# JuliaReinforcementLearning/ReinforcementLearning.jl

Measured on NVIDIA H100. Metric: env-steps/sec at 65536 CartPole envs (full PPO iteration: rollout T=32 + GAE + 4 epochs x 4 minibatches), higher is better.
Workload: dtype f32

## Files before the change

### reinforcementlearning.jl_b200/csrc/nn_tc.cu

```cuda
#include "nn.cuh"
#include "perm.cuh"
#include "policy.cuh"
#include "tc_fwd.cuh"
#include "tc_split.h"
#include "wgmma.cuh"

namespace {

using tcfwd::G_F;
using tcfwd::GW_S;
using tcfwd::WIMG_BYTES;
using tcfwd::split2;
using tcfwd::wimg_off;
constexpr int TM = tcfwd::TM;
constexpr int H = tcfwd::H;
constexpr float kScaleW = tcfwd::kScale;

constexpr int NT7 = 512;
constexpr int kMaxStage = 10;
constexpr int GF_T = 128;
constexpr int GS_T = 16 * GF_T;
constexpr int FIMG = 8 * GS_T;
constexpr float kScaleH = 64.0f, kScaleX = 64.0f;
constexpr int kNo = 2;

struct SmemBwd {
    static_assert(FIMG % 128 == 0 && WIMG_BYTES % 128 == 0 && (2 * GS_T) % 16 == 0, "operand images must stay 128-byte aligned");
    alignas(128) uint8_t FP_full[FIMG];
    alignas(128) uint8_t FP_lo[FIMG];
    alignas(128) uint8_t FH_lo[FIMG];
    alignas(128) uint8_t FH_full[FIMG];
    alignas(128) uint8_t FQ_full[FIMG];
    alignas(128) uint8_t FQ_lo[FIMG];
    alignas(128) uint8_t B1[WIMG_BYTES];
    alignas(128) uint8_t XT[2][2 * GS_T];
    alignas(128) uint8_t AH_full[FIMG];
    alignas(128) uint8_t AH_lo[FIMG];
    alignas(16) float D[TM * H];
    uint64_t H1pos[2][TM];
    float W1[kInMax * H];
    float b1[H], b2[H];
    float W3[H * kNo];
    float b3[kNo];
    float Zp[4 * kNo * TM];
    float Red[32];
    double RedD[16];
    float step_scale;
    alignas(8) uint64_t bar1;
    alignas(8) uint64_t bar3;
    alignas(8) uint64_t bar4;
    float AccW2[64 * 65 + 64];
    float AccD4[64 * 9];
};
__device__ __forceinline__ int d_off(int s, int col) { return s * H + ((((col >> 2) ^ (s & 15))) << 2) + (col & 3); }
__device__ __forceinline__ void d_ld16(const float* D, int s, int f0, float (&v)[16]) {
#pragma unroll
    for (int u = 0; u < 4; ++u) {
        const float4 q4 = *reinterpret_cast<const float4*>(D + d_off(s, f0 + 4 * u));
        v[4 * u] = q4.x; v[4 * u + 1] = q4.y; v[4 * u + 2] = q4.z; v[4 * u + 3] = q4.w;
    }
}
template <int TB>
__device__ __forceinline__ void gemm_ts3(float (&d)[32], const uint8_t* a_hi, const uint8_t* a_lo, int h, uint64_t dB, uint32_t b_step) {
    const uint64_t dA = wg::make_desc(wg::smem_u32(a_hi) + 8 * h * GF_T, GS_T, GF_T), dAl = wg::make_desc(wg::smem_u32(a_lo) + 8 * h * GF_T, GS_T, GF_T);
    wg::fence();
#pragma unroll
    for (int k = 0; k < 4; ++k) {
        const uint32_t aa = k * 2 * GS_T, bb = k * b_step;
        wg::mma_m64n64k16<0, TB>(d, wg::desc_add(dA, aa), wg::desc_add(dB, bb), k ? 1u : 0u);
        wg::mma_m64n64k16<0, TB>(d, wg::desc_add(dA, aa), wg::desc_add(dB, 8 * GW_S + bb), 1u);
        wg::mma_m64n64k16<0, TB>(d, wg::desc_add(dAl, aa), wg::desc_add(dB, bb), 1u);
    }
    wg::commit();
    wg::wait_all();
}
__device__ __forceinline__ uint32_t fimg_off(int f, int s) { return (uint32_t)((f >> 3) * GS_T + (s >> 3) * GF_T + (s & 7) * 16 + (f & 7) * 2); }
__device__ __forceinline__ void store16_feat(uint8_t* img, int f0, int s, const uint32_t (&v)[8]) {
    uint8_t* p = img + fimg_off(f0, s);
    *reinterpret_cast<uint4*>(p) = make_uint4(v[0], v[1], v[2], v[3]);
    *reinterpret_cast<uint4*>(p + GS_T) = make_uint4(v[4], v[5], v[6], v[7]);
}
using b200perm::perm_index;
using b200perm::perm_index_bits;

__device__ __forceinline__ float lane_transpose_reduce32(float (&v)[32], int lane) {
#pragma unroll
    for (int st = 0; st < 5; ++st) {
        const int half = 16 >> st, off = 16 >> st;
        const bool upper = (lane & off) != 0;
#pragma unroll
        for (int n = 0; n < half; ++n) {
            float send = upper ? v[n] : v[n + half];
            float keep = upper ? v[n + half] : v[n];
            v[n] = keep + __shfl_xor_sync(0xffffffffu, send, off);
        }
    }
    return v[0];
}

__device__ __forceinline__ void worker_sync() { asm volatile("bar.sync 1, 512;" ::: "memory"); }
__device__ __forceinline__ void group_sync(int q) { asm volatile("bar.sync %0, 128;" ::"r"(5 + q) : "memory"); }
__device__ __forceinline__ void ready_arrive(int id) { asm volatile("bar.arrive %0, 640;" ::"r"(id) : "memory"); }
__device__ __forceinline__ void ready_wait(int id) { asm volatile("bar.sync %0, 640;" ::"r"(id) : "memory"); }
#ifdef B200RL_K7_TIMING
__device__ unsigned long long g_k7_phase[40];
__device__ int g_k7_watch = 0;
#define K7_T(i) do { if (tid == (g_k7_watch & 0xFFFF) && (int)blockIdx.x == (g_k7_watch >> 16)) { long long now_ = clock64(); g_k7_phase[i] += (unsigned long long)(now_ - tprev_); tprev_ = now_; } } while (0)
#else
#define K7_T(i) do { } while (0)
#endif
constexpr int NT7_ALL = NT7 + 128;
constexpr int kRegsMma = 64, kRegsWorker = 104;
static_assert(128 * kRegsMma + NT7 * kRegsWorker <= NT7_ALL * 96, "setmaxnreg split must fit the CTA's register allocation");
constexpr int kBarRdyA = 2, kBarRdyB = 3;
constexpr int kBarMma = 4;
__device__ __forceinline__ void mma_sync() { asm volatile("bar.sync %0, 128;" ::"n"(kBarMma) : "memory"); }

template <int ACT>
__global__ void __launch_bounds__(NT7_ALL, 1)
ac_loss_grad_tc_kernel(MlpDesc actor, MlpDesc critic, const float* params , AcHyper hp, AcBatch b, float* partial,
                       float* __restrict__ loss_partial, int64_t np_total, float scale_base ,
                       OptStep st ,
                       int n_actor ) {
    extern __shared__ __align__(1024) unsigned char smem_raw[];
    SmemBwd& sm = *reinterpret_cast<SmemBwd*>(smem_raw);
    const int role = (int)blockIdx.x < n_actor ? 0 : 1;
    const int cta = role ? (int)blockIdx.x - n_actor : (int)blockIdx.x;
    const int nctas = role ? (int)gridDim.x - n_actor : n_actor;
    const int nrows = max(n_actor, (int)gridDim.x - n_actor);
    const float scale_p = scale_base * (role ? 4.0f : 64.0f);
    const MlpDesc d = role ? critic : actor;
    const int act = ACT >= 0 ? ACT : d.act;
    const bool relu = act == B200RL_ACT_RELU;
    const int64_t poff = role ? actor.nparams() : 0;
    const float* __restrict__ p = params + poff;
    const int tid = threadIdx.x, warp = tid >> 5, lane = tid & 31;
    const int q = warp & 3, c = (warp >> 2) & 3;
    const int s = 32 * q + lane;
    {
        const float* b1 = p + (int64_t)H * d.in;
        const float* W2 = b1 + H;
        const float* b2 = W2 + (int64_t)H * H;
        const float s1 = relu ? kScaleH : 1.0f;
        for (int k = tid; k < kInMax * H; k += NT7_ALL) sm.W1[k] = (k / H) < d.in ? p[k] * s1 : 0.f;
        for (int k = tid; k < H; k += NT7_ALL) { sm.b1[k] = b1[k] * s1; sm.b2[k] = b2[k]; }
        for (int k = tid; k < H * kNo; k += NT7_ALL) {
            int j = k / kNo, o = k % kNo;
            sm.W3[k] = o < d.nout ? p[head_w<false>(d, o, j)] : 0.f;
        }
        if (tid < kNo) sm.b3[tid] = tid < d.nout ? p[head_b<false>(d, tid)] : 0.f;
        tcfwd::fill_w2_image<NT7_ALL>(sm.B1, W2);
    }
    if (tid == 32) {
        wg::mbar_init(&sm.bar1, 128); wg::mbar_init(&sm.bar3, 128); wg::mbar_init(&sm.bar4, 128);
    }
    wg::fence_proxy_async();
    __syncthreads();
    const float inv_s1 = 1.0f / (kScaleH * kScaleW), inv_s3 = 1.0f / (scale_p * kScaleH), inv_sp = 1.0f / scale_p, inv_s4 = 1.0f / (scale_p * kScaleX);
    const int64_t ntiles = (b.B + TM - 1) / TM;

    if (warp >= NT7 / 32) {
        asm volatile("setmaxnreg.dec.sync.aligned.u32 %0;" ::"n"(kRegsMma));
        const int t = tid - NT7, row0 = 16 * (t >> 5) + ((t & 31) >> 2), col0 = 2 * (t & 3);
        const uint64_t dB1k = wg::make_desc(wg::smem_u32(sm.B1), G_F, GW_S);
        const uint64_t dB1t = wg::make_desc(wg::smem_u32(sm.B1), GW_S, G_F);
        float dacc[32];
        auto store_d = [&](int h) {
#pragma unroll
            for (int j = 0; j < 8; ++j)
#pragma unroll
                for (int hh = 0; hh < 2; ++hh)
                    *reinterpret_cast<float2*>(sm.D + d_off(64 * h + row0 + 8 * hh, 8 * j + col0)) = make_float2(dacc[4 * j + 2 * hh], dacc[4 * j + 2 * hh + 1]);
        };
        auto gemm1 = [&](int h) { gemm_ts3<0>(dacc, sm.AH_full, sm.AH_lo, h, dB1k, 2 * G_F); };
        auto gemm2 = [&](int h) { gemm_ts3<1>(dacc, sm.FP_full, sm.FP_lo, h, dB1t, 2 * GW_S); };
        auto store_dp1 = [&](int h, int pbuf) {
#pragma unroll
            for (int hh = 0; hh < 2; ++hh) {
                const int ss = 64 * h + row0 + 8 * hh;
                const uint64_t pos = relu ? sm.H1pos[pbuf][ss] >> col0 : 0u;
#pragma unroll
                for (int j = 0; j < 8; ++j) {
                    const uint32_t off = fimg_off(8 * j + col0, ss);
                    float v0 = dacc[4 * j + 2 * hh] * (1.0f / kScaleW), v1 = dacc[4 * j + 2 * hh + 1] * (1.0f / kScaleW);
                    if (relu) {
                        v0 = ((pos >> (8 * j)) & 1u) ? v0 : 0.f;
                        v1 = ((pos >> (8 * j + 1)) & 1u) ? v1 : 0.f;
                    } else {
                        const float inv_h = 1.0f / kScaleH;
                        const float2 hf = __half22float2(*reinterpret_cast<const __half2*>(sm.FH_full + off));
                        const float2 lf = __half22float2(*reinterpret_cast<const __half2*>(sm.FH_lo + off));
                        v0 *= dact_f(act, (hf.x + lf.x) * inv_h);
                        v1 *= dact_f(act, (hf.y + lf.y) * inv_h);
                    }
                    uint32_t hi, lo;
                    split2(v0, v1, hi, lo);
                    *reinterpret_cast<uint32_t*>(sm.FQ_full + off) = hi;
                    *reinterpret_cast<uint32_t*>(sm.FQ_lo + off) = lo;
                }
            }
        };
        auto gemm3 = [&](int buf) {
            const uint64_t dPh = wg::make_desc(wg::smem_u32(sm.FP_full), GF_T, GS_T), dPl = wg::make_desc(wg::smem_u32(sm.FP_lo), GF_T, GS_T);
            const uint64_t dHh = wg::make_desc(wg::smem_u32(sm.FH_full), GF_T, GS_T), dHl = wg::make_desc(wg::smem_u32(sm.FH_lo), GF_T, GS_T);
            wg::fence();
#pragma unroll
            for (int k = 0; k < 8; ++k) {
                const uint32_t a = k * 2 * GF_T;
                wg::mma_m64n64k16<1, 1>(dacc, wg::desc_add(dPh, a), wg::desc_add(dHh, a), k ? 1u : 0u);
                wg::mma_m64n64k16<1, 1>(dacc, wg::desc_add(dPl, a), wg::desc_add(dHh, a), 1u);
                wg::mma_m64n64k16<1, 1>(dacc, wg::desc_add(dPh, a), wg::desc_add(dHl, a), 1u);
            }
            wg::commit();
            wg::wait_all();
#pragma unroll
            for (int j = 0; j < 8; ++j)
#pragma unroll
                for (int hh = 0; hh < 2; ++hh)
#pragma unroll
                    for (int e = 0; e < 2; ++e) sm.AccW2[(row0 + 8 * hh) * 65 + 8 * j + col0 + e] += dacc[4 * j + 2 * hh + e];
            const uint64_t dX = wg::make_desc(wg::smem_u32(sm.XT[buf]), GF_T, GS_T);
            float d8[4] = {0.f, 0.f, 0.f, 0.f};
            wg::fence();
#pragma unroll
            for (int k = 0; k < 8; ++k) {
                const uint32_t a = k * 2 * GF_T;
                wg::mma_m64n8k16<1, 1>(d8, wg::desc_add(dPh, a), wg::desc_add(dX, a), k ? 1u : 0u);
                wg::mma_m64n8k16<1, 1>(d8, wg::desc_add(dPl, a), wg::desc_add(dX, a), 1u);
            }
            wg::commit();
            wg::wait_all();
            if (col0 == 4) {
                sm.AccW2[64 * 65 + row0] += d8[0];
                sm.AccW2[64 * 65 + row0 + 8] += d8[2];
            }
        };
        auto gemm4 = [&](int buf) {
            const uint64_t dQh = wg::make_desc(wg::smem_u32(sm.FQ_full), GF_T, GS_T), dQl = wg::make_desc(wg::smem_u32(sm.FQ_lo), GF_T, GS_T);
            const uint64_t dX = wg::make_desc(wg::smem_u32(sm.XT[buf]), GF_T, GS_T);
            float d4[4] = {0.f, 0.f, 0.f, 0.f};
            wg::fence();
#pragma unroll
            for (int k = 0; k < 8; ++k) {
                const uint32_t a = k * 2 * GF_T;
                wg::mma_m64n8k16<1, 1>(d4, wg::desc_add(dQh, a), wg::desc_add(dX, a), k ? 1u : 0u);
                wg::mma_m64n8k16<1, 1>(d4, wg::desc_add(dQh, a), wg::desc_add(dX, GS_T + a), 1u);
                wg::mma_m64n8k16<1, 1>(d4, wg::desc_add(dQl, a), wg::desc_add(dX, a), 1u);
            }
            wg::commit();
            wg::wait_all();
#pragma unroll
            for (int hh = 0; hh < 2; ++hh)
#pragma unroll
                for (int e = 0; e < 2; ++e)
                    if (col0 + e < 5) sm.AccD4[(row0 + 8 * hh) * 9 + col0 + e] += d4[2 * hh + e];
        };
        if (cta < ntiles) {
            ready_wait(kBarRdyB);
            for (int h = 0; h < 2; ++h) { gemm1(h); store_d(h); }
            wg::mbar_arrive(&sm.bar1);
        }
        int buf = 0;
        for (int64_t tile = cta; tile < ntiles; tile += nctas, buf ^= 1) {
            ready_wait(kBarRdyA);
            for (int h = 0; h < 2; ++h) { gemm2(h); store_dp1(h, buf); }
            wg::fence_proxy_async();
            if (tile + nctas < ntiles) {
                ready_wait(kBarRdyB);
                for (int h = 0; h < 2; ++h) { gemm1(h); store_d(h); }
                wg::mbar_arrive(&sm.bar1);
            }
            gemm3(buf);
            wg::mbar_arrive(&sm.bar3);
            mma_sync();
            gemm4(buf);
            wg::mbar_arrive(&sm.bar4);
        }
    } else {
    asm volatile("setmaxnreg.inc.sync.aligned.u32 %0;" ::"n"(kRegsWorker));
    float g3[2][16];
    float gb3a0 = 0.f, gb3a1 = 0.f;
#pragma unroll
    for (int k = 0; k < 16; ++k) { g3[0][k] = 0.f; g3[1][k] = 0.f; }
    float l0 = 0.f, l1 = 0.f;
    float mean = 0.f, inv_std = 1.f;
    if (hp.normalize_adv && b.norm2) { mean = b.norm2[0]; inv_std = b.norm2[1]; }
    uint32_t ph1 = 0, ph3 = 0, ph4 = 0;
    bool gemm4_pending = false;
    int xbuf = 0;
    int pbuf = 0;
#ifdef B200RL_K7_TIMING
    long long tprev_ = clock64();
#endif
    const int pbits = b200perm::perm_bits(b.perm_n);
    const uint32_t pkey = ac_perm_key(b);
    auto index_of = [&](int64_t t) -> int32_t {
        const int64_t j = t * TM + s;
        if (t >= ntiles || j >= b.B) return -1;
        return b.idx ? b.idx[j] : (int32_t)perm_index_bits((uint32_t)(b.perm_offset + j), b.perm_n, pkey, pbits);
    };
    auto request = [&](int32_t g, float (&x)[kInMax], float (&a)[4]) {
#pragma unroll
        for (int k = 0; k < kInMax; ++k) { x[k] = 0.f; a[k] = 0.f; }
        if (g < 0) return;
        if (b.rec) {
            const float4 v0 = b.rec[2 * (int64_t)g], v1 = b.rec[2 * (int64_t)g + 1];
            x[0] = v0.x; x[1] = v0.y; x[2] = v0.z; x[3] = v0.w;
            a[0] = v1.x; a[1] = v1.y; a[2] = v1.z; a[3] = v1.w;
        } else {
#pragma unroll
            for (int i = 0; i < kInMax; ++i)
                if (i < b.ns) x[i] = b.states[(int64_t)b.ns * g + i];
            a[0] = reinterpret_cast<const float*>(b.actions)[g];
            a[1] = b.logp_old ? b.logp_old[g] : 0.f;
            a[2] = b.adv[g];
            a[3] = b.ret[g];
        }
    };
    float pfx[kInMax] = {0.f, 0.f, 0.f, 0.f}, pfa[4] = {0.f, 0.f, 0.f, 0.f};
    float aux[4] = {0.f, 0.f, 0.f, 0.f};
    int32_t gi_next = -1;
    bool gemm3_pending = false;
    float* const out = partial + (int64_t)cta * np_total + poff;
    float* const gW1 = out;
    float* const gb1 = out + (int64_t)H * d.in;
    float* const gW2 = gb1 + H;
    float* const gb2 = gW2 + (int64_t)H * H;
    for (int k = tid; k < 64 * 65 + 64; k += NT7) sm.AccW2[k] = 0.f;
    for (int k = tid; k < 64 * 9; k += NT7) sm.AccD4[k] = 0.f;
    float xo[kInMax];
    auto publish = [&](int64_t t) {
#pragma unroll
        for (int i = 0; i < kInMax; ++i) xo[i] = pfx[i];
        aux[0] = pfa[0];
        aux[1] = role == 0 ? pfa[1] : 0.f;
        aux[2] = role == 0 ? (hp.normalize_adv ? (pfa[2] - mean) * inv_std : pfa[2]) : 0.f;
        aux[3] = role == 0 ? 0.f : pfa[3];
        if (c == 0) {
            uint32_t h01, l01, h23, l23;
            split2(xo[0] * kScaleX, xo[1] * kScaleX, h01, l01);
            split2(xo[2] * kScaleX, xo[3] * kScaleX, h23, l23);
            uint8_t* xt = sm.XT[xbuf] + fimg_off(0, s);
            *reinterpret_cast<uint4*>(xt) = make_uint4(h01, h23, 0x3C00u, 0u);
            *reinterpret_cast<uint4*>(xt + GS_T) = make_uint4(l01, l23, 0u, 0u);
        }
        K7_T(16);
        xbuf ^= 1;
        request(gi_next, pfx, pfa);
        gi_next = index_of(t + 2 * nctas);
        K7_T(17);
    };
    auto layer1 = [&]() {
        uint32_t pos = 0;
        uint32_t hi8[8], lo8[8];
#pragma unroll
        for (int ch = 0; ch < 4; ++ch) {
            const int f0 = 16 * c + 4 * ch;
            float4 bb = *reinterpret_cast<const float4*>(sm.b1 + f0);
            float h[4] = {bb.x, bb.y, bb.z, bb.w};
#pragma unroll
            for (int k = 0; k < kInMax; ++k) {
                float4 w = *reinterpret_cast<const float4*>(sm.W1 + k * H + f0);
                h[0] = fmaf(w.x, xo[k], h[0]); h[1] = fmaf(w.y, xo[k], h[1]); h[2] = fmaf(w.z, xo[k], h[2]); h[3] = fmaf(w.w, xo[k], h[3]);
            }
            if (relu) {
#pragma unroll
                for (int e = 0; e < 4; ++e) { pos |= (h[e] > 0.f ? 1u : 0u) << (4 * ch + e); h[e] = fmaxf(h[e], 0.f); }
            } else {
#pragma unroll
                for (int e = 0; e < 4; ++e) h[e] = act_f(act, h[e]) * kScaleH;
            }
            split2(h[0], h[1], hi8[2 * ch], lo8[2 * ch]);
            split2(h[2], h[3], hi8[2 * ch + 1], lo8[2 * ch + 1]);
        }
        if (relu) reinterpret_cast<uint16_t*>(&sm.H1pos[pbuf][s])[c] = (uint16_t)pos;
        pbuf ^= 1;
        store16_feat(sm.AH_full, 16 * c, s, hi8);
        store16_feat(sm.AH_lo, 16 * c, s, lo8);
    };
    if (cta < ntiles) {
        request(index_of(cta), pfx, pfa);
        gi_next = index_of(cta + nctas);
        publish(cta);
        layer1();
        wg::fence_proxy_async();
        ready_arrive(kBarRdyB);
    }
#ifdef B200RL_K7_TIMING
    tprev_ = clock64();
#endif
    for (int64_t tile = cta; tile < ntiles; tile += nctas) {
        const bool has_next = tile + nctas < ntiles;
        wg::mbar_wait(&sm.bar1, ph1);
        ph1 ^= 1u;
        K7_T(0);
        float h2[16];
        {
            float v[16];
            d_ld16(sm.D, s, 16 * c, v);
            float zp[kNo] = {0.f, 0.f};
#pragma unroll
            for (int k = 0; k < 16; ++k) {
                const int f = 16 * c + k;
                h2[k] = act_f(act, fmaf(v[k], inv_s1, sm.b2[f]));
                float2 w = *reinterpret_cast<const float2*>(sm.W3 + f * kNo);
                zp[0] = fmaf(w.x, h2[k], zp[0]); zp[1] = fmaf(w.y, h2[k], zp[1]);
            }
#pragma unroll
            for (int o = 0; o < kNo; ++o) sm.Zp[(c * kNo + o) * TM + s] = zp[o];
        }
        K7_T(1);
        group_sync(q);
        K7_T(2);
        {
            float z[kNo];
#pragma unroll
            for (int o = 0; o < kNo; ++o)
                z[o] = sm.b3[o] + ((sm.Zp[o * TM + s] + sm.Zp[(kNo + o) * TM + s]) + (sm.Zp[(2 * kNo + o) * TM + s] + sm.Zp[(3 * kNo + o) * TM + s]));
            const bool valid = (tile * TM + s) < b.B;
            const policy::LossOut<kNo> lo_ = policy::sample_loss(actor.heads2, actor.nout, role, hp, b.inv_B, z, aux[0], aux[1], aux[2], aux[3]);
            float dz[kNo];
#pragma unroll
            for (int o = 0; o < kNo; ++o) dz[o] = valid ? lo_.dz[o] : 0.f;
            if (c == 0 && valid) { l0 += lo_.l0; l1 += lo_.l1; gb3a0 += dz[0]; gb3a1 += dz[1]; }
            const float dzs0 = dz[0] * scale_p, dzs1 = dz[1] * scale_p;
            float dp[16];
#pragma unroll
            for (int k = 0; k < 16; ++k) {
                const int f = 16 * c + k;
                float2 w = *reinterpret_cast<const float2*>(sm.W3 + f * kNo);
                const float dh = fmaf(w.x, dzs0, w.y * dzs1);
                dp[k] = relu ? (h2[k] > 0.f ? dh : 0.f) : dh * (1.f - h2[k] * h2[k]);
                g3[0][k] = fmaf(dz[0], h2[k], g3[0][k]);
                g3[1][k] = fmaf(dz[1], h2[k], g3[1][k]);
            }
            uint32_t hi8[8], lo8[8];
#pragma unroll
            for (int m = 0; m < 8; ++m) split2(dp[2 * m], dp[2 * m + 1], hi8[m], lo8[m]);
            K7_T(3);
            if (gemm3_pending) {
                wg::mbar_wait(&sm.bar3, ph3);
                ph3 ^= 1u;
                gemm3_pending = false;
            }
            K7_T(4);
            store16_feat(sm.FP_full, 16 * c, s, hi8);
            store16_feat(sm.FP_lo, 16 * c, s, lo8);
            {
                const uint32_t off = fimg_off(16 * c, s);
                const uint4 h0 = *reinterpret_cast<const uint4*>(sm.AH_full + off), h1 = *reinterpret_cast<const uint4*>(sm.AH_full + off + GS_T);
                const uint4 l0 = *reinterpret_cast<const uint4*>(sm.AH_lo + off), l1 = *reinterpret_cast<const uint4*>(sm.AH_lo + off + GS_T);
                *reinterpret_cast<uint4*>(sm.FH_full + off) = h0; *reinterpret_cast<uint4*>(sm.FH_full + off + GS_T) = h1;
                *reinterpret_cast<uint4*>(sm.FH_lo + off) = l0; *reinterpret_cast<uint4*>(sm.FH_lo + off + GS_T) = l1;
            }
        }
        K7_T(5);
        wg::fence_proxy_async();
        if (gemm4_pending) {
            wg::mbar_wait(&sm.bar4, ph4);
            ph4 ^= 1u;
        }
        K7_T(6);
        ready_arrive(kBarRdyA);
        gemm3_pending = true;
        gemm4_pending = true;
        K7_T(7);
        if (has_next) {
            publish(tile + nctas);
            layer1();
            wg::fence_proxy_async();
            K7_T(8);
            ready_arrive(kBarRdyB);
            K7_T(9);
        }
#ifdef B200RL_K7_TIMING
        if (tid == (g_k7_watch & 0xFFFF) && (int)blockIdx.x == (g_k7_watch >> 16)) g_k7_phase[15] += 1;
#endif
    }
    if (gemm3_pending) wg::mbar_wait(&sm.bar3, ph3);
    if (gemm4_pending) wg::mbar_wait(&sm.bar4, ph4);
    worker_sync();
    for (int k = tid; k < H * H; k += NT7) gW2[k] = sm.AccW2[(k & 63) * 65 + (k >> 6)] * inv_s3;
    if (tid < H) {
        gb2[tid] = sm.AccW2[64 * 65 + tid] * inv_sp;
        gb1[tid] = sm.AccD4[tid * 9 + 4] * inv_sp;
        for (int i = 0; i < d.in; ++i) gW1[tid + H * i] = sm.AccD4[tid * 9 + i] * inv_s4;
    }
    if (cta >= (int)gridDim.x - nctas) {
        const int64_t ooff = role ? 0 : actor.nparams(), on = role ? actor.nparams() : critic.nparams();
        float* orow = partial + (int64_t)cta * np_total + ooff;
        for (int64_t kk = tid; kk < on; kk += NT7) orow[kk] = 0.f;
    }
    float* red = reinterpret_cast<float*>(sm.FP_full);
    static_assert(offsetof(SmemBwd, XT) - offsetof(SmemBwd, FP_full) >= (2 * TM * 65 + 2 * 8 * 64) * 4, "drain scratch");
    {
        constexpr int RS = 65;
        float* seg = red + 2 * TM * RS;
#pragma unroll
        for (int k = 0; k < 16; ++k) {
            red[0 * TM * RS + s * RS + 16 * c + k] = g3[0][k];
            red[1 * TM * RS + s * RS + 16 * c + k] = g3[1][k];
        }
        worker_sync();
        {
            const int col = tid & 63, g = tid >> 6;
#pragma unroll
            for (int m = 0; m < 2; ++m) {
                float a = 0.f;
#pragma unroll
                for (int ss = 0; ss < 16; ++ss) a += red[m * TM * RS + (16 * g + ss) * RS + col];
                seg[(m * 8 + g) * 64 + col] = a;
            }
        }
        worker_sync();
        if (tid < 2 * H) {
            const int m = tid >> 6, col = tid & 63;
            float a = 0.f;
#pragma unroll
            for (int g = 0; g < 8; ++g) a += seg[(m * 8 + g) * 64 + col];
            if (m < d.nout) out[head_w<false>(d, m, col)] = a;
        }
        worker_sync();
    }
    if (c == 0) { red[s] = gb3a0; red[TM + s] = gb3a1; }
    worker_sync();
    if (warp < d.nout) {
        float a = (red[warp * TM + lane] + red[warp * TM + 32 + lane]) + (red[warp * TM + 64 + lane] + red[warp * TM + 96 + lane]);
#pragma unroll
        for (int o = 16; o > 0; o >>= 1) a += __shfl_xor_sync(0xffffffffu, a, o);
        if (lane == 0) out[head_b<false>(d, warp)] = a;
    }
    float t0 = l0, t1 = l1;
#pragma unroll
    for (int o = 16; o > 0; o >>= 1) { t0 += __shfl_xor_sync(0xffffffffu, t0, o); t1 += __shfl_xor_sync(0xffffffffu, t1, o); }
    worker_sync();
    if (lane == 0) { sm.Red[warp] = t0; sm.Red[16 + warp] = t1; }
    worker_sync();
    if (tid == 0) {
        float a0 = 0.f, a1 = 0.f;
        for (int k = 0; k < 16; ++k) { a0 += sm.Red[k]; a1 += sm.Red[16 + k]; }
        float* lp = loss_partial + (int64_t)blockIdx.x * 4;
        lp[0] = role ? 0.f : a0; lp[1] = role ? 0.f : a1; lp[2] = role ? a0 : 0.f; lp[3] = 0.f;
    }
    if (blockIdx.x == 0)
        for (int k = tid; k < 4 * (2 * nrows - (int)gridDim.x); k += NT7) loss_partial[4 * (int64_t)gridDim.x + k] = 0.f;
    if (st.params) {
        const unsigned int G = gridDim.x;
        K7_T(24);
        worker_sync();
        K7_T(25);
        if (tid == 0) optim::grid_barrier(st.counters, G);
        worker_sync();
        K7_T(26);
        const int per = (int)((np_total + G - 1) / G);
        const int64_t k = (int64_t)blockIdx.x * per + tid;
        const bool mine = tid < per && k < np_total;
        const unsigned int seq = st.tab.nranks > 1 ? *st.seq_ptr + 1u : 0u;
        float* stage = reinterpret_cast<float*>(sm.FP_full);
        const int nstage = per * nrows;
        const int64_t k0 = (int64_t)blockIdx.x * per;
        {
            float t[kMaxStage];
#pragma unroll
            for (int j = 0; j < kMaxStage; ++j) {
                const int e = tid + j * NT7;
                const int row = e / per, col = e - row * per;
                t[j] = (e < nstage && k0 + col < np_total) ? __ldcg(partial + (int64_t)row * np_total + k0 + col) : 0.f;
            }
#pragma unroll
            for (int j = 0; j < kMaxStage; ++j) {
                const int e = tid + j * NT7;
                if (e < nstage) stage[e] = t[j];
            }
        }
        float* lstage = stage + nstage;
        if (blockIdx.x == 0) {
            float t[2];
#pragma unroll
            for (int j = 0; j < 2; ++j) t[j] = tid + j * NT7 < 4 * (int)G ? __ldcg(loss_partial + tid + j * NT7) : 0.f;
#pragma unroll
            for (int j = 0; j < 2; ++j) if (tid + j * NT7 < 4 * (int)G) lstage[tid + j * NT7] = t[j];
        }
        float m_k = 0.f, v_k = 0.f, p_k = 0.f;
        if (mine) { m_k = st.m[k]; v_k = st.v[k]; p_k = st.params[k]; }
        worker_sync();
        K7_T(27);
        float gk = 0.f;
        if (mine) {
            for (int c0 = 0; c0 < nrows; c0 += 8) {
                float t[8];
#pragma unroll
                for (int j = 0; j < 8; ++j) t[j] = c0 + j < nrows ? stage[(c0 + j) * per + tid] : 0.f;
#pragma unroll
                for (int j = 0; j < 8; ++j) if (c0 + j < nrows) gk += t[j];
            }
        }
        float lsum = 0.f;
        const bool loss_thread = blockIdx.x == 0 && tid < 4;
        if (loss_thread) {
            for (unsigned int c0 = 0; c0 < G; c0 += 8) {
                float t[8];
#pragma unroll
                for (int j = 0; j < 8; ++j) t[j] = c0 + j < G ? lstage[(c0 + j) * 4 + tid] : 0.f;
#pragma unroll
                for (int j = 0; j < 8; ++j) if (c0 + j < G) lsum += t[j];
            }
        }
        if (st.tab.nranks > 1) {
            const unsigned slot = seq & 1u;
            if (mine) p2p_push(st.tab, 0, slot, (size_t)k, __float_as_uint(gk), seq);
            if (loss_thread) p2p_push(st.tab, 0, slot, (size_t)np_total + tid, __float_as_uint(lsum), seq);
            if (mine) gk = p2p_sum_ranks(st.tab, 0, slot, (size_t)k, gk, seq);
            if (loss_thread) lsum = p2p_sum_ranks(st.tab, 0, slot, (size_t)np_total + tid, lsum, seq);
        }
        if (loss_thread) optim::publish_loss(st, tid, lsum);
        double sq = (double)gk * (double)gk;
#pragma unroll
        for (int o = 16; o > 0; o >>= 1) sq += __shfl_xor_sync(0xffffffffu, sq, o);
        if (lane == 0) sm.RedD[warp] = sq;
        worker_sync();
        K7_T(28);
        if (warp == 0) {
            if (lane == 0) {
                double t = 0.0;
                for (int w = 0; w < NT7 / 32; ++w) t += sm.RedD[w];
                st.cta_sumsq[blockIdx.x] = t;
                optim::grid_barrier(st.counters + 1, G);
            }
            __syncwarp();
            K7_T(29);
            double part[8];
#pragma unroll
            for (int j = 0; j < 8; ++j) part[j] = (unsigned)(lane + 32 * j) < G ? __ldcg(st.cta_sumsq + lane + 32 * j) : 0.0;
            double tot = 0.0;
#pragma unroll
            for (int j = 0; j < 8; ++j) tot += part[j];
#pragma unroll
            for (int o = 16; o > 0; o >>= 1) tot += __shfl_xor_sync(0xffffffffu, tot, o);
            if (lane == 0) {
                const float gn = (float)sqrt(tot);
                sm.step_scale = optim::clip_scale(gn, st.max_norm);
                if (blockIdx.x == 0) optim::publish_gnorm(st, gn);
            }
        }
        worker_sync();
        K7_T(30);
        const float bt1 = st.beta_t[0], bt2 = st.beta_t[1];
        if (mine) {
            gk *= sm.step_scale;
            st.grad[k] = gk;
            const optim::AdamOut a = optim::adam_update(gk, m_k, v_k, p_k, st.lr, st.b1, st.b2, st.eps, bt1, bt2);
            st.m[k] = a.m; st.v[k] = a.v; st.params[k] = a.p;
        }
        worker_sync();
        if (tid == 0) optim::close_step<3>(st, bt1, bt2, st.tab.nranks > 1, seq);
        K7_T(31);
    }
    }
    __syncthreads();
}

}

int nn_tc_actor_ctas(int grid, const MlpDesc& actor, const AcHyper& hp, int64_t ntiles) {
    static int forced = -2;
    if (forced == -2) { const char* e = getenv("B200RL_K7_ACTOR_CTAS"); forced = e ? atoi(e) : -1; }
    if (forced > 0 && forced < grid) return forced;
    (void)hp;
    return b200rl_tc_actor_ctas(grid, actor.heads2 != 0, ntiles);
}
int nn_tc_partial_rows(int grid, const MlpDesc& actor, const AcHyper& hp, int64_t B) {
    const int na = nn_tc_actor_ctas(grid, actor, hp, (B + TM - 1) / TM);
    return na > grid - na ? na : grid - na;
}
bool nn_tc_bwd_supported(const MlpDesc& actor, const MlpDesc& critic) {
    return actor.H == 64 && critic.H == 64 && actor.in <= kInMax && actor.nout <= 2 && critic.nout == 1;
}
bool nn_tc_step_fits(b200rl_ctx* ctx, int grid, const MlpDesc& actor, const AcHyper& hp, int64_t B, int64_t np) {
    const int64_t per = (np + grid - 1) / grid;
    return grid <= ctx->sm_count && grid <= 256 && per <= NT7 && per * nn_tc_partial_rows(grid, actor, hp, B) <= kMaxStage * NT7 &&
           4 * grid <= 2 * NT7;
}
int nn_tc_ac_loss_grad(b200rl_ctx* ctx, int grid, const MlpDesc& actor, const MlpDesc& critic, const float* params, const AcHyper& hp,
                       const AcBatch& b, float* partial, float* loss_partial, int64_t np, const OptStep* step) {
    const OptStep st = step ? *step : OptStep{};
    const int n_actor = nn_tc_actor_ctas(grid, actor, hp, (b.B + TM - 1) / TM);
    size_t smem = sizeof(SmemBwd) + 128;
    static unsigned long long attr_devices = 0;
    if (first_use_on_device(attr_devices, ctx->device)) {
        CUDA_TRY(cudaFuncSetAttribute(ac_loss_grad_tc_kernel<B200RL_ACT_RELU>, cudaFuncAttributeMaxDynamicSharedMemorySize, (int)smem));
        CUDA_TRY(cudaFuncSetAttribute(ac_loss_grad_tc_kernel<B200RL_ACT_TANH>, cudaFuncAttributeMaxDynamicSharedMemorySize, (int)smem));
        CUDA_TRY(cudaFuncSetAttribute(ac_loss_grad_tc_kernel<-1>, cudaFuncAttributeMaxDynamicSharedMemorySize, (int)smem));
    }
    const float scale_base = exp2f(floorf(log2f(1.0f / b.inv_B)));
    if (actor.act == critic.act && actor.act == B200RL_ACT_RELU)
        ac_loss_grad_tc_kernel<B200RL_ACT_RELU><<<grid, NT7_ALL, smem, ctx->stream>>>(actor, critic, params, hp, b, partial, loss_partial, np, scale_base, st, n_actor);
    else if (actor.act == critic.act && actor.act == B200RL_ACT_TANH)
        ac_loss_grad_tc_kernel<B200RL_ACT_TANH><<<grid, NT7_ALL, smem, ctx->stream>>>(actor, critic, params, hp, b, partial, loss_partial, np, scale_base, st, n_actor);
    else
        ac_loss_grad_tc_kernel<-1><<<grid, NT7_ALL, smem, ctx->stream>>>(actor, critic, params, hp, b, partial, loss_partial, np, scale_base, st, n_actor);
    LAUNCH_CHECK(ctx);
    return B200RL_OK;
}

#ifdef B200RL_K7_TIMING
extern "C" int b200rl_debug_k7_watch(int tid) {
    cudaDeviceSynchronize();
    return cudaMemcpyToSymbol(g_k7_watch, &tid, sizeof tid) == cudaSuccess ? 0 : -1;
}
extern "C" int b200rl_debug_k7_phases(unsigned long long* out16, int reset) {
    cudaDeviceSynchronize();
    if (cudaMemcpyFromSymbol(out16, g_k7_phase, sizeof(unsigned long long) * 40) != cudaSuccess) return -1;
    if (reset) { unsigned long long z[24] = {0}; cudaMemcpyToSymbol(g_k7_phase, z, sizeof z); }
    return 0;
}
#endif
```

Before: 308.3 million.

## Double-buffer layer-1 activation images and split MMA handoff barriers per half-tile

```diff
diff --git a/reinforcementlearning.jl_b200/csrc/nn_tc.cu b/reinforcementlearning.jl_b200/csrc/nn_tc.cu
--- a/reinforcementlearning.jl_b200/csrc/nn_tc.cu
+++ b/reinforcementlearning.jl_b200/csrc/nn_tc.cu
@@ -28,14 +28,11 @@
     static_assert(FIMG % 128 == 0 && WIMG_BYTES % 128 == 0 && (2 * GS_T) % 16 == 0, "operand images must stay 128-byte aligned");
     alignas(128) uint8_t FP_full[FIMG];
     alignas(128) uint8_t FP_lo[FIMG];
-    alignas(128) uint8_t FH_lo[FIMG];
-    alignas(128) uint8_t FH_full[FIMG];
+    alignas(128) uint8_t AH[2][2][FIMG];
     alignas(128) uint8_t FQ_full[FIMG];
     alignas(128) uint8_t FQ_lo[FIMG];
     alignas(128) uint8_t B1[WIMG_BYTES];
     alignas(128) uint8_t XT[2][2 * GS_T];
-    alignas(128) uint8_t AH_full[FIMG];
-    alignas(128) uint8_t AH_lo[FIMG];
     alignas(16) float D[TM * H];
     uint64_t H1pos[2][TM];
     float W1[kInMax * H];
@@ -46,7 +43,7 @@
     float Red[32];
     double RedD[16];
     float step_scale;
-    alignas(8) uint64_t bar1;
+    alignas(8) uint64_t bar1[2];
     alignas(8) uint64_t bar3;
     alignas(8) uint64_t bar4;
     float AccW2[64 * 65 + 64];
@@ -100,8 +97,8 @@
 
 __device__ __forceinline__ void worker_sync() { asm volatile("bar.sync 1, 512;" ::: "memory"); }
 __device__ __forceinline__ void group_sync(int q) { asm volatile("bar.sync %0, 128;" ::"r"(5 + q) : "memory"); }
-__device__ __forceinline__ void ready_arrive(int id) { asm volatile("bar.arrive %0, 640;" ::"r"(id) : "memory"); }
-__device__ __forceinline__ void ready_wait(int id) { asm volatile("bar.sync %0, 640;" ::"r"(id) : "memory"); }
+__device__ __forceinline__ void ready_arrive(int id) { asm volatile("bar.arrive %0, 384;" ::"r"(id) : "memory"); }
+__device__ __forceinline__ void ready_wait(int id) { asm volatile("bar.sync %0, 384;" ::"r"(id) : "memory"); }
 #ifdef B200RL_K7_TIMING
 __device__ unsigned long long g_k7_phase[40];
 __device__ int g_k7_watch = 0;
@@ -112,7 +109,7 @@
 constexpr int NT7_ALL = NT7 + 128;
 constexpr int kRegsMma = 64, kRegsWorker = 104;
 static_assert(128 * kRegsMma + NT7 * kRegsWorker <= NT7_ALL * 96, "setmaxnreg split must fit the CTA's register allocation");
-constexpr int kBarRdyA = 2, kBarRdyB = 3;
+constexpr int kBarRdyA = 2, kBarRdyB = 9;
 constexpr int kBarMma = 4;
 __device__ __forceinline__ void mma_sync() { asm volatile("bar.sync %0, 128;" ::"n"(kBarMma) : "memory"); }
 
@@ -137,6 +134,7 @@
     const int tid = threadIdx.x, warp = tid >> 5, lane = tid & 31;
     const int q = warp & 3, c = (warp >> 2) & 3;
     const int s = 32 * q + lane;
+    const int half = q >> 1;
     {
         const float* b1 = p + (int64_t)H * d.in;
         const float* W2 = b1 + H;
@@ -152,7 +150,7 @@
         tcfwd::fill_w2_image<NT7_ALL>(sm.B1, W2);
     }
     if (tid == 32) {
-        wg::mbar_init(&sm.bar1, 128); wg::mbar_init(&sm.bar3, 128); wg::mbar_init(&sm.bar4, 128);
+        wg::mbar_init(&sm.bar1[0], 128); wg::mbar_init(&sm.bar1[1], 128); wg::mbar_init(&sm.bar3, 128); wg::mbar_init(&sm.bar4, 128);
     }
     wg::fence_proxy_async();
     __syncthreads();
@@ -172,7 +170,7 @@
                 for (int hh = 0; hh < 2; ++hh)
                     *reinterpret_cast<float2*>(sm.D + d_off(64 * h + row0 + 8 * hh, 8 * j + col0)) = make_float2(dacc[4 * j + 2 * hh], dacc[4 * j + 2 * hh + 1]);
         };
-        auto gemm1 = [&](int h) { gemm_ts3<0>(dacc, sm.AH_full, sm.AH_lo, h, dB1k, 2 * G_F); };
+        auto gemm1 = [&](int h, int buf) { gemm_ts3<0>(dacc, sm.AH[buf][0], sm.AH[buf][1], h, dB1k, 2 * G_F); };
         auto gemm2 = [&](int h) { gemm_ts3<1>(dacc, sm.FP_full, sm.FP_lo, h, dB1t, 2 * GW_S); };
         auto store_dp1 = [&](int h, int pbuf) {
 #pragma unroll
@@ -188,8 +186,8 @@
                         v1 = ((pos >> (8 * j + 1)) & 1u) ? v1 : 0.f;
                     } else {
                         const float inv_h = 1.0f / kScaleH;
-                        const float2 hf = __half22float2(*reinterpret_cast<const __half2*>(sm.FH_full + off));
-                        const float2 lf = __half22float2(*reinterpret_cast<const __half2*>(sm.FH_lo + off));
+                        const float2 hf = __half22float2(*reinterpret_cast<const __half2*>(sm.AH[pbuf][0] + off));
+                        const float2 lf = __half22float2(*reinterpret_cast<const __half2*>(sm.AH[pbuf][1] + off));
                         v0 *= dact_f(act, (hf.x + lf.x) * inv_h);
                         v1 *= dact_f(act, (hf.y + lf.y) * inv_h);
                     }
@@ -202,7 +200,7 @@
         };
         auto gemm3 = [&](int buf) {
             const uint64_t dPh = wg::make_desc(wg::smem_u32(sm.FP_full), GF_T, GS_T), dPl = wg::make_desc(wg::smem_u32(sm.FP_lo), GF_T, GS_T);
-            const uint64_t dHh = wg::make_desc(wg::smem_u32(sm.FH_full), GF_T, GS_T), dHl = wg::make_desc(wg::smem_u32(sm.FH_lo), GF_T, GS_T);
+            const uint64_t dHh = wg::make_desc(wg::smem_u32(sm.AH[buf][0]), GF_T, GS_T), dHl = wg::make_desc(wg::smem_u32(sm.AH[buf][1]), GF_T, GS_T);
             wg::fence();
 #pragma unroll
             for (int k = 0; k < 8; ++k) {
@@ -256,20 +254,25 @@
                     if (col0 + e < 5) sm.AccD4[(row0 + 8 * hh) * 9 + col0 + e] += d4[2 * hh + e];
         };
         if (cta < ntiles) {
-            ready_wait(kBarRdyB);
-            for (int h = 0; h < 2; ++h) { gemm1(h); store_d(h); }
-            wg::mbar_arrive(&sm.bar1);
+            for (int h = 0; h < 2; ++h) {
+                ready_wait(kBarRdyB + h);
+                gemm1(h, 0); store_d(h);
+                wg::mbar_arrive(&sm.bar1[h]);
+            }
         }
         int buf = 0;
         for (int64_t tile = cta; tile < ntiles; tile += nctas, buf ^= 1) {
-            ready_wait(kBarRdyA);
-            for (int h = 0; h < 2; ++h) { gemm2(h); store_dp1(h, buf); }
+            const bool has_next = tile + nctas < ntiles;
+            for (int h = 0; h < 2; ++h) {
+                ready_wait(kBarRdyA + h);
+                gemm2(h); store_dp1(h, buf);
+                if (has_next) {
+                    ready_wait(kBarRdyB + h);
+                    gemm1(h, buf ^ 1); store_d(h);
+                    wg::mbar_arrive(&sm.bar1[h]);
+                }
+            }
             wg::fence_proxy_async();
-            if (tile + nctas < ntiles) {
-                ready_wait(kBarRdyB);
-                for (int h = 0; h < 2; ++h) { gemm1(h); store_d(h); }
-                wg::mbar_arrive(&sm.bar1);
-            }
             gemm3(buf);
             wg::mbar_arrive(&sm.bar3);
             mma_sync();
@@ -374,9 +377,9 @@
             split2(h[2], h[3], hi8[2 * ch + 1], lo8[2 * ch + 1]);
         }
         if (relu) reinterpret_cast<uint16_t*>(&sm.H1pos[pbuf][s])[c] = (uint16_t)pos;
+        store16_feat(sm.AH[pbuf][0], 16 * c, s, hi8);
+        store16_feat(sm.AH[pbuf][1], 16 * c, s, lo8);
         pbuf ^= 1;
-        store16_feat(sm.AH_full, 16 * c, s, hi8);
-        store16_feat(sm.AH_lo, 16 * c, s, lo8);
     };
     if (cta < ntiles) {
         request(index_of(cta), pfx, pfa);
@@ -384,14 +387,14 @@
         publish(cta);
         layer1();
         wg::fence_proxy_async();
-        ready_arrive(kBarRdyB);
+        ready_arrive(kBarRdyB + half);
     }
 #ifdef B200RL_K7_TIMING
     tprev_ = clock64();
 #endif
     for (int64_t tile = cta; tile < ntiles; tile += nctas) {
         const bool has_next = tile + nctas < ntiles;
-        wg::mbar_wait(&sm.bar1, ph1);
+        wg::mbar_wait(&sm.bar1[half], ph1);
         ph1 ^= 1u;
         K7_T(0);
         float h2[16];
@@ -446,13 +449,6 @@
             K7_T(4);
             store16_feat(sm.FP_full, 16 * c, s, hi8);
             store16_feat(sm.FP_lo, 16 * c, s, lo8);
-            {
-                const uint32_t off = fimg_off(16 * c, s);
-                const uint4 h0 = *reinterpret_cast<const uint4*>(sm.AH_full + off), h1 = *reinterpret_cast<const uint4*>(sm.AH_full + off + GS_T);
-                const uint4 l0 = *reinterpret_cast<const uint4*>(sm.AH_lo + off), l1 = *reinterpret_cast<const uint4*>(sm.AH_lo + off + GS_T);
-                *reinterpret_cast<uint4*>(sm.FH_full + off) = h0; *reinterpret_cast<uint4*>(sm.FH_full + off + GS_T) = h1;
-                *reinterpret_cast<uint4*>(sm.FH_lo + off) = l0; *reinterpret_cast<uint4*>(sm.FH_lo + off + GS_T) = l1;
-            }
         }
         K7_T(5);
         wg::fence_proxy_async();
@@ -461,7 +457,7 @@
             ph4 ^= 1u;
         }
         K7_T(6);
-        ready_arrive(kBarRdyA);
+        ready_arrive(kBarRdyA + half);
         gemm3_pending = true;
         gemm4_pending = true;
         K7_T(7);
@@ -470,7 +466,7 @@
             layer1();
             wg::fence_proxy_async();
             K7_T(8);
-            ready_arrive(kBarRdyB);
+            ready_arrive(kBarRdyB + half);
             K7_T(9);
         }
 #ifdef B200RL_K7_TIMING
```

Measured after the change: 321.5 million, median of 6. 1.04x the previous value.
